# zhirui-gao/PoseProbe

Measured on AMD Instinct MI355X. Metric: rays_per_sec_train_step, higher is better.
Workload: dtype f32 (3xf16-split products); 1 GPU; DTU-scan1-like 3-view 400x400, object-branch train step (ray select, render, losses, backward, TV+Adam), 160^3 grid, 186 samples/ray, N_rand=1024/GPU; per-step ray permutation + jitter pre-generated on the host and resident in HBM (the reference draws randperm inside the step); grid=160, n_rand_per_gpu=1024, samples_in_bbox_last_step=57637, parallelism=single GPU

## Files before the change

poseprobe_amd/csrc/pp_gemm_tn_tr.h:

```cpp
#pragma once
#include "pp_gemm_split.h"

#ifndef TN_DBG
#define TN_DBG 0
#endif
__device__ __forceinline__ int tn_off(int row, int ch) { return 256 * row + 16 * (ch ^ (((row & 3) << 2) | ((row >> 2) & 3))); }

#ifdef TN_TIMERS
#define TN_TIMERS_ON 1
__device__ unsigned long long g_tn_t[8];
extern "C" int pp_debug_read_tn_timers(unsigned long long* out8, int reset) {
  if (hipMemcpyFromSymbol(out8, HIP_SYMBOL(g_tn_t), sizeof(g_tn_t)) != hipSuccess) return 1;
  if (reset) { unsigned long long z[8] = {0}; if (hipMemcpyToSymbol(HIP_SYMBOL(g_tn_t), z, sizeof(z)) != hipSuccess) return 1; }
  return 0;
}
#endif
static __global__ __launch_bounds__(256, 2) void k_gemm_tn_tr(const float* __restrict__ Y_, int ldy, const float* __restrict__ X_, int ldx,
                                                          int Kx_, float* __restrict__ Wbar_, int ldwb, float* __restrict__ bbar_,
                                                          const int32_t* __restrict__ count, int rcap,
                                                          const float* __restrict__ y_max, const float* __restrict__ x_max) {
  constexpr int CH = 64;
  __shared__ __attribute__((aligned(1024))) unsigned char img[4 * CH * 256];
  unsigned char* const Yh = img;
  unsigned char* const Yl = img + CH * 256;
  unsigned char* const Xh = img + 2 * CH * 256;
  unsigned char* const Xl = img + 3 * CH * 256;
  const int nkb = (Kx_ + 127) >> 7;
  const int nb = blockIdx.y / nkb, kb = blockIdx.y - nb * nkb;
  const float* __restrict__ Y = Y_ + nb * 128;
  const float* __restrict__ X = X_ + kb * 128;
  const int Kx = min(128, Kx_ - kb * 128);
  float* __restrict__ Wbar = Wbar_ + (size_t)nb * 128 * ldwb + kb * 128;
  float* __restrict__ bbar = (bbar_ && kb == 0) ? bbar_ + nb * 128 : nullptr;
  const int R = min(count[0], rcap);
  const int rows_per_wg = ((R + (int)gridDim.x - 1) / (int)gridDim.x + CH - 1) / CH * CH;
  const int rb = blockIdx.x * rows_per_wg;
  if (rb >= R) return;
  const int re = min(rb + rows_per_wg, R);
  const int tid = threadIdx.x, lane = tid & 63, wid = tid >> 6;
  const int wr = wid >> 1, wc = wid & 1;
  const int l31 = lane & 31, lh = lane >> 5;
  const float sY = pp_split_scale(y_max[0]), sX = pp_split_scale(x_max[0]);
  const int c4 = tid & 31, rblk = tid >> 5;
  const int kx4 = Kx >> 2;
  f32x16 acc[2][2];
#pragma unroll
  for (int t = 0; t < 2; ++t)
#pragma unroll
    for (int u = 0; u < 2; ++u)
#pragma unroll
      for (int i = 0; i < 16; ++i) acc[t][u][i] = 0.f;
  float bsum[4] = {0.f, 0.f, 0.f, 0.f};
  float4 ry[8], rx[8];
  auto load_rows = [&](int r0, int i0, int i1) {
#pragma unroll
    for (int i = 0; i < 8; ++i) {
      if (i < i0 || i >= i1) continue;
      const int gr = min(r0 + rblk * 8 + i, R - 1);
      ry[i] = *reinterpret_cast<const float4*>(Y + (size_t)gr * ldy + c4 * 4);
      if (TN_DBG & 4) rx[i] = ry[i];
      else rx[i] = *reinterpret_cast<const float4*>(X + (size_t)gr * ldx + (c4 < kx4 ? c4 : 0) * 4);
    }
  };
  typedef __fp16 tn_h4 __attribute__((vector_size(8)));
  const int fg = lane >> 4, fq = (lane & 15) >> 2, fp = lane & 3;
  auto frag = [&](const unsigned char* plane, int cb, int ks) -> pp_half8 {
    const int ch = ((cb + 16 * (fg & 1)) >> 3) + (fp >> 1);
    const int row = ks + 8 * (fg >> 1) + fq;
    const tn_h4 a = __builtin_amdgcn_ds_read_tr16_b64_v4f16((__attribute__((address_space(3))) tn_h4*)(plane + tn_off(row, ch) + 8 * (fp & 1)));
    const tn_h4 b = __builtin_amdgcn_ds_read_tr16_b64_v4f16((__attribute__((address_space(3))) tn_h4*)(plane + tn_off(row + 4, ch) + 8 * (fp & 1)));
    typedef __fp16 tn_h8 __attribute__((vector_size(16)));
    const tn_h8 v = __builtin_shufflevector(a, b, 0, 1, 2, 3, 4, 5, 6, 7);
    return __builtin_bit_cast(pp_half8, v);
  };
#ifdef TN_TIMERS_ON
  unsigned long long tsum[8] = {0}, tprev = __builtin_readcyclecounter();
#define TN_TICK(i) do { const unsigned long long t__ = __builtin_readcyclecounter(); tsum[i] += t__ - tprev; tprev = t__; } while (0)
#else
#define TN_TICK(i) do {} while (0)
#endif
  load_rows(rb, 0, 8);
  for (int r0 = rb; r0 < re; r0 += CH) {
    asm volatile("s_waitcnt vmcnt(0)" ::: "memory");
    TN_TICK(0);
#pragma unroll
    for (int i = 0; i < 8; ++i) {
      const int o = tn_off(rblk * 8 + i, c4 >> 1) + 8 * (c4 & 1);
      const float ky = (r0 + rblk * 8 + i < re) ? 1.f : 0.f, kx = (c4 < kx4) ? ky : 0.f;
      ry[i].x *= ky; ry[i].y *= ky; ry[i].z *= ky; ry[i].w *= ky;
      rx[i].x *= kx; rx[i].y *= kx; rx[i].z *= kx; rx[i].w *= kx;
      pp_half4 h, l;
      pp_split4(ry[i], sY, h, l);
      *reinterpret_cast<pp_half4*>(Yh + o) = h;
      *reinterpret_cast<pp_half4*>(Yl + o) = l;
      pp_split4(rx[i], sX, h, l);
      *reinterpret_cast<pp_half4*>(Xh + o) = h;
      *reinterpret_cast<pp_half4*>(Xl + o) = l;
    }
    if (bbar) {
#pragma unroll
      for (int i = 0; i < 8; ++i) { bsum[0] += ry[i].x; bsum[1] += ry[i].y; bsum[2] += ry[i].z; bsum[3] += ry[i].w; }
    }
    TN_TICK(1);
    __syncthreads();
    TN_TICK(2);
    if (wc * 64 < Kx) {
      pp_half8 fa[2][4], fb[2][4];
      auto fetch = [&](int par, int ks) {
#pragma unroll
        for (int t = 0; t < 2; ++t) { fa[par][2 * t] = frag(Yh, wr * 64 + t * 32, ks); fa[par][2 * t + 1] = frag(Yl, wr * 64 + t * 32, ks); }
#pragma unroll
        for (int u = 0; u < 2; ++u) { fb[par][2 * u] = frag(Xh, wc * 64 + u * 32, ks); fb[par][2 * u + 1] = frag(Xl, wc * 64 + u * 32, ks); }
      };
      fetch(0, 0);
#pragma unroll
      for (int s4 = 0; s4 < CH / 16; ++s4) {
        const int par = s4 & 1;
        if (s4 + 1 < CH / 16 && !(TN_DBG & 2)) fetch(par ^ 1, (s4 + 1) * 16);
        if (TN_DBG & 2) { for (int i = 0; i < 4; ++i) { fa[par ^ 1][i] = fa[par][i]; fb[par ^ 1][i] = fb[par][i]; } }
#pragma unroll
        for (int t = 0; t < 2; ++t) {
#pragma unroll
          for (int u = 0; u < 2; ++u) {
            acc[t][u] = __builtin_amdgcn_mfma_f32_32x32x16_f16(fa[par][2 * t + 1], fb[par][2 * u], acc[t][u], 0, 0, 0);
            acc[t][u] = __builtin_amdgcn_mfma_f32_32x32x16_f16(fa[par][2 * t], fb[par][2 * u + 1], acc[t][u], 0, 0, 0);
            acc[t][u] = __builtin_amdgcn_mfma_f32_32x32x16_f16(fa[par][2 * t], fb[par][2 * u], acc[t][u], 0, 0, 0);
          }
          if (t == 0 && !(TN_DBG & 1)) {
            __builtin_amdgcn_sched_barrier(0);
            load_rows(r0 + CH, 2 * s4, 2 * s4 + 2);
            __builtin_amdgcn_sched_barrier(0);
          }
        }
      }
    } else if (!(TN_DBG & 1)) {
      load_rows(r0 + CH, 0, 8);
    }
    TN_TICK(3);
    __syncthreads();
    TN_TICK(4);
  }
  const float inv = 1.0f / (sY * sX);
  if (wc * 64 < Kx) {
#pragma unroll
    for (int t = 0; t < 2; ++t)
#pragma unroll
      for (int u = 0; u < 2; ++u) {
        const int k = wc * 64 + u * 32 + l31;
        if (k >= Kx) continue;
#pragma unroll
        for (int reg = 0; reg < 16; ++reg) {
          const int n = wr * 64 + t * 32 + (reg & 3) + 8 * (reg >> 2) + 4 * lh;
          atomicAdd(&Wbar[(size_t)n * ldwb + k], acc[t][u][reg] * inv);
        }
      }
  }
  if (bbar) {
    float* red = reinterpret_cast<float*>(img);
#pragma unroll
    for (int j = 0; j < 4; ++j) red[rblk * 128 + c4 * 4 + j] = bsum[j];
    __syncthreads();
    if (tid < 128) {
      float sum = 0.f;
#pragma unroll
      for (int q = 0; q < 8; ++q) sum += red[q * 128 + tid];
      atomicAdd(&bbar[tid], sum);
    }
  }
#ifdef TN_TIMERS_ON
  TN_TICK(5);
  if (tid == 0)
    for (int i = 0; i < 8; ++i) atomicAdd(&g_tn_t[i], tsum[i]);
#endif
#undef TN_TICK
}
```

poseprobe_amd/csrc/pp_mlp_split.hip:

```cpp
#include "pp_common.h"
#include "pp_mlp_fused.h"
#include "pp_gemm_split.h"

typedef float f32x4 __attribute__((ext_vector_type(4)));

#define LDA 132
#define TILE_ROWS 64
#define LDH2 136
#define PLANE (TILE_ROWS * LDH2)
#ifndef MS_DBG
#define MS_DBG 0
#endif
#ifdef MS_TIMERS
__device__ unsigned long long g_ms_t[16];
extern "C" int pp_debug_read_timers(unsigned long long* out16, int reset) {
  if (hipMemcpyFromSymbol(out16, HIP_SYMBOL(g_ms_t), sizeof(g_ms_t)) != hipSuccess) return 1;
  if (reset) { unsigned long long z[16] = {0}; if (hipMemcpyToSymbol(HIP_SYMBOL(g_ms_t), z, sizeof(z)) != hipSuccess) return 1; }
  return 0;
}
#define TICK(i) do { const unsigned long long t__ = __builtin_readcyclecounter(); tsum[i] += t__ - tprev; tprev = t__; } while (0)
#else
#define TICK(i) do {} while (0)
#endif
#define PP_WAIT_VMEM() do { __builtin_amdgcn_s_waitcnt(0x0F70); asm volatile("" ::: "memory"); } while (0)

namespace {

struct SplitW { pp_half8 h[8], l[8]; };

__device__ __forceinline__ float wave_max(float v) {
#pragma unroll
  for (int o = 32; o > 0; o >>= 1) v = fmaxf(v, __shfl_xor(v, o, 64));
  return v;
}
__device__ __forceinline__ float block_max(float v, float* red, int tid, int& phase) {
  float* set = red + 16 * (phase & 1);
  ++phase;
  v = fmaxf(v, __int_as_float(__builtin_amdgcn_update_dpp(0, __float_as_int(v), 0xB1, 0xf, 0xf, true)));
  v = fmaxf(v, __int_as_float(__builtin_amdgcn_update_dpp(0, __float_as_int(v), 0x4E, 0xf, 0xf, true)));
  v = fmaxf(v, __int_as_float(__builtin_amdgcn_update_dpp(0, __float_as_int(v), 0x141, 0xf, 0xf, true)));
  v = fmaxf(v, __int_as_float(__builtin_amdgcn_update_dpp(0, __float_as_int(v), 0x140, 0xf, 0xf, true)));
  if ((tid & 15) == 0) set[tid >> 4] = v;
  __syncthreads();
  const float4 a = *reinterpret_cast<const float4*>(set), b = *reinterpret_cast<const float4*>(set + 4),
               c = *reinterpret_cast<const float4*>(set + 8), d = *reinterpret_cast<const float4*>(set + 12);
  return fmaxf(fmaxf(fmaxf(fmaxf(a.x, a.y), fmaxf(a.z, a.w)), fmaxf(fmaxf(b.x, b.y), fmaxf(b.z, b.w))),
               fmaxf(fmaxf(fmaxf(c.x, c.y), fmaxf(c.z, c.w)), fmaxf(fmaxf(d.x, d.y), fmaxf(d.z, d.w))));
}
__device__ __forceinline__ int scale_exp(float mx) {
  if (!(mx > 0.f) || !(mx < 3.0e38f)) return 0;
  int e;
  frexpf(mx, &e);
  return min(max(15 - e, -60), 60);
}
__device__ __forceinline__ float pow2(int e) { return ldexpf(1.f, e); }
__device__ __forceinline__ float tile_scale(float mx) { return pow2(scale_exp(mx)); }
__device__ __forceinline__ void split1(float x, _Float16& h, _Float16& l) {
  h = (_Float16)x;
  l = (_Float16)(x - (float)h);
}
__device__ __forceinline__ void split8(const float4& a, const float4& b, float s, pp_half8& h, pp_half8& l) {
  const float v[8] = {a.x * s, a.y * s, a.z * s, a.w * s, b.x * s, b.y * s, b.z * s, b.w * s};
#pragma unroll
  for (int i = 0; i < 8; ++i) {
    _Float16 hh, ll;
    split1(v[i], hh, ll);
    h[i] = hh; l[i] = ll;
  }
}
__device__ __forceinline__ float amax4(const float4& v) { return fmaxf(fmaxf(fabsf(v.x), fabsf(v.y)), fmaxf(fabsf(v.z), fabsf(v.w))); }
__device__ __forceinline__ float asum4(const float4& v) { return (fabsf(v.x) + fabsf(v.y)) + (fabsf(v.z) + fabsf(v.w)); }

__device__ __forceinline__ int load_w_rows_split(SplitW& w, float& l1, const float* __restrict__ W, int n, int lh, float* red,
                                                   int tid, int& phase) {
  float4 v[16];
  float mx = 0.f, sum = 0.f;
#pragma unroll
  for (int ks = 0; ks < 8; ++ks) {
    v[2 * ks] = *reinterpret_cast<const float4*>(W + (size_t)n * 128 + 16 * ks + 8 * lh);
    v[2 * ks + 1] = *reinterpret_cast<const float4*>(W + (size_t)n * 128 + 16 * ks + 8 * lh + 4);
    mx = fmaxf(mx, fmaxf(amax4(v[2 * ks]), amax4(v[2 * ks + 1])));
    sum += asum4(v[2 * ks]) + asum4(v[2 * ks + 1]);
  }
  sum += __shfl_xor(sum, 32, 64);
  const int e = scale_exp(block_max(mx, red, tid, phase));
  const float s = pow2(e);
  l1 = block_max(sum, red, tid, phase) * 1.0001f;
#pragma unroll
  for (int ks = 0; ks < 8; ++ks) split8(v[2 * ks], v[2 * ks + 1], s, w.h[ks], w.l[ks]);
  return e;
}

struct NoHook { __device__ __forceinline__ void operator()(int) const {} };
template <int KS = 8, int LD = LDH2, int PL = PLANE, class Hook = NoHook>
__device__ __forceinline__ void mma_half(const _Float16* __restrict__ rows, const SplitW& w, f32x16& acc, int l31, int lh,
                                         Hook hook = Hook()) {
  const _Float16* p = rows + l31 * LD + 8 * lh;
  pp_half8 h = *reinterpret_cast<const pp_half8*>(p), l = *reinterpret_cast<const pp_half8*>(p + PL);
#pragma unroll
  for (int ks = 0; ks < (MS_DBG == 1 ? 0 : KS); ++ks) {
    pp_half8 nh = h, nl = l;
    if (ks + 1 < KS) {
      nh = *reinterpret_cast<const pp_half8*>(p + 16 * (ks + 1));
      nl = *reinterpret_cast<const pp_half8*>(p + 16 * (ks + 1) + PL);
    }
    acc = __builtin_amdgcn_mfma_f32_32x32x16_f16(w.h[ks], l, acc, 0, 0, 0);
    acc = __builtin_amdgcn_mfma_f32_32x32x16_f16(w.l[ks], h, acc, 0, 0, 0);
    acc = __builtin_amdgcn_mfma_f32_32x32x16_f16(w.h[ks], h, acc, 0, 0, 0);
    h = nh; l = nl;
    hook(ks);
  }
}

__device__ __forceinline__ void zero16(f32x16& acc) {
#pragma unroll
  for (int i = 0; i < 16; ++i) acc[i] = 0.f;
}

typedef _Float16 half2_t __attribute__((ext_vector_type(2)));

template <int COLS, bool SPLIT>
struct HalfEpilogue {
  float4 b[4];
  float y[16];
  float p[16];
  unsigned h[8], l[8];
  float xmax;
  __device__ __forceinline__ void begin(const float* __restrict__ brow) {
    xmax = 0.f;
#pragma unroll
    for (int q = 0; q < 4; ++q) b[q] = *reinterpret_cast<const float4*>(brow + 8 * q);
  }
  __device__ __forceinline__ void step(int i, const f32x16& acc, float inv, float snext, bool ok, float* __restrict__ Crow,
                                       _Float16* __restrict__ Arow) {
    __builtin_amdgcn_sched_barrier(0);
    if (i == 0) {
#pragma unroll
      for (int q = 0; q < 4; ++q) {
        y[4 * q] = fmaf(acc[4 * q], inv, b[q].x); y[4 * q + 1] = fmaf(acc[4 * q + 1], inv, b[q].y);
        y[4 * q + 2] = fmaf(acc[4 * q + 2], inv, b[q].z); y[4 * q + 3] = fmaf(acc[4 * q + 3], inv, b[q].w);
      }
    } else if (i == 1) {
      if (COLS == 4) {
#pragma unroll
        for (int e = 0; e < 16; ++e)
          asm("v_mov_b32_dpp %0, %1 quad_perm:[0,0,0,0] row_mask:0xf bank_mask:0xf bound_ctrl:1" : "=v"(p[e]) : "v"(y[e]));
#pragma unroll
        for (int e = 0; e < 16; ++e) asm("v_ashrrev_i32 %0, 31, %1" : "=v"(p[e]) : "v"(p[e]));
      }
    } else if (i == 2) {
#pragma unroll
      for (int e = 0; e < 16; ++e) {
        if (COLS == 4) asm("v_bfi_b32 %0, %1, 0, %2" : "=v"(y[e]) : "v"(p[e]), "v"(y[e]));
        else y[e] = fmaxf(y[e], 0.f);
      }
// ... 896 lines not shown
    const int r0 = t * TILE_ROWS;
    float gl = 0.f;
    if (tid < 192) {
      const int m = tid / 3, o = tid - 3 * m;
      const float r = RG[b][0][tid];
      gl = (r0 + m < R) ? RG[b][1][tid] * r * (1.f - r) : 0.f;
      GL[m * 4 + o] = gl;
      if (logit_grad && r0 + m < R) logit_grad[(size_t)(r0 + m) * lg_ld + o] = gl;
    } else {
      GL[(tid - 192) * 4 + 3] = 0.f;
    }
    slot_max(&Mx[b][4], fabsf(gl), lane);
  };
  auto w3_accumulate = [&]() {
    const float* __restrict__ xs = &XS[(h0 * 32) * 128 + j0];
#pragma unroll 8
    for (int r = 0; r < 32; ++r) {
      const float4 g = *reinterpret_cast<const float4*>(&GL[(h0 * 32 + r) * 4]);
      const float x = xs[r * 128];
      wacc3[0] = fmaf(g.x, x, wacc3[0]); wacc3[1] = fmaf(g.y, x, wacc3[1]); wacc3[2] = fmaf(g.z, x, wacc3[2]);
      if (j0 < 3) bacc3 += GL[(h0 * 32 + r) * 4 + j0];
    }
  };
  int e2n = 0;
  auto out_layer_bwd = [&](int t, int b, _Float16* dst) {
    const float gmx = slot_get(&Mx[b][4]);
    const int eg = scale_exp(gmx);
    const int e2 = scale_exp(gmx * w3l1);
    const float sg = pow2(eg), s2 = pow2(e2), inv = pow2(-(eg + ew3)), n2 = pow2(-e2);
    const int r0 = t * TILE_ROWS;
    float* crow = ybar + (size_t)(r0 + l31) * 128 + fb;
    HalfEpilogueB<true> eb;
#pragma unroll
    for (int hh = 0; hh < 2; ++hh) {
      float4 x = *reinterpret_cast<const float4*>(&GL[(hh * 32 + l31) * 4]);
      if (lh != 0) x = make_float4(0.f, 0.f, 0.f, 0.f);
      pp_half8 xh, xl;
      split8(x, make_float4(0.f, 0.f, 0.f, 0.f), sg, xh, xl);
      f32x16 a;
      zero16(a);
      a = __builtin_amdgcn_mfma_f32_32x32x16_f16(a3h, xl, a, 0, 0, 0);
      a = __builtin_amdgcn_mfma_f32_32x32x16_f16(a3l, xh, a, 0, 0, 0);
      a = __builtin_amdgcn_mfma_f32_32x32x16_f16(a3h, xh, a, 0, 0, 0);
      eb.begin(&XS[(hh * 32 + l31) * 128 + fb]);
      eb.all(a, inv, s2, r0 + hh * 32 + l31 < R, crow + hh * 32 * 128, dst + (hh * 32 + l31) * LDH2 + fb);
      slot_max(&Mx[b][hh], eb.vmax(n2), lane);
    }
    e2n = e2;
  };

  if (tid < 16) Mx[tid >> 3][tid & 7] = 0u;
  stage(blockIdx.x, 0);
  __builtin_amdgcn_s_waitcnt(0);
  __syncthreads();
  logit_grads(blockIdx.x, 0);
  __syncthreads();
  w3_accumulate();
  out_layer_bwd(blockIdx.x, 0, At[0]);
  __syncthreads();

  int par = 0;
  for (int tile = blockIdx.x; tile < ntiles; tile += gridDim.x, par ^= 1) {
    const int r0 = tile * TILE_ROWS;
    const int tnext = tile + gridDim.x;
    const bool more = tnext < ntiles;
    const bool ok0 = r0 + l31 < R, ok1 = r0 + 32 + l31 < R;
    _Float16* const Aa = At[par];
    _Float16* const Ab = At[par ^ 1];
    const int e2 = e2n;
    float* const crow = ybar + (size_t)(r0 + l31) * 128 + fb;
    f32x16 acc0, acc1;
    HalfEpilogueB<true> eb;
    if (tid < 5) Mx[par ^ 1][tid] = 0u;
    if (more) stage(tnext, par ^ 1);
    stage_tile(H1, r0, GT);
    zero16(acc0);
    mma_half(Aa, w2, acc0, l31, lh);
    PP_WAIT_VMEM();
    __syncthreads();
    const int e10 = scale_exp(slot_get(&Mx[par][0]) * l1_2), e11 = scale_exp(slot_get(&Mx[par][1]) * l1_2);
    zero16(acc1);
    eb.begin(&GT[l31 * 128 + fb]);
    mma_half(Aa + 32 * LDH2, w2, acc1, l31, lh, [&](int ks) {
      eb.step(ks, acc0, pow2(-(e2 + ew2)), pow2(e10), ok0, crow + LS, Ab + l31 * LDH2 + fb);
    });
    slot_max(&Mx[par][2], eb.vmax(pow2(-e10)), lane);
    __syncthreads();
    zero16(acc0);
    eb.begin(&GT[(32 + l31) * 128 + fb]);
    mma_half(Ab, w1, acc0, l31, lh, [&](int ks) {
      eb.step(ks, acc1, pow2(-(e2 + ew2)), pow2(e11), ok1, crow + LS + 32 * 128, Ab + (32 + l31) * LDH2 + fb);
    });
    slot_max(&Mx[par][3], eb.vmax(pow2(-e11)), lane);
    __syncthreads();
    stage_tile(H0, r0, GT);
    zero16(acc1);
    mma_half(Ab + 32 * LDH2, w1, acc1, l31, lh);
    PP_WAIT_VMEM();
    __syncthreads();
    const int e00 = scale_exp(slot_get(&Mx[par][2]) * l1_1), e01 = scale_exp(slot_get(&Mx[par][3]) * l1_1);
    eb.begin(&GT[l31 * 128 + fb]);
    eb.all(acc0, pow2(-(e10 + ew1)), pow2(e00), ok0, crow + 2 * LS, Aa + l31 * LDH2 + fb);
    eb.begin(&GT[(32 + l31) * 128 + fb]);
    eb.all(acc1, pow2(-(e11 + ew1)), pow2(e01), ok1, crow + 2 * LS + 32 * 128, Aa + (32 + l31) * LDH2 + fb);
    if (more) logit_grads(tnext, par ^ 1);
    __syncthreads();
    {
      f32x16 fa;
      zero16(fa);
      mma_half(Aa + rb * 32 * LDH2, w0, fa, l31, lh);
      const float inv = pow2(-((rb ? e01 : e00) + ew0));
      const int row = r0 + rb * 32 + l31;
      if (row < R) {
        float* __restrict__ ft = feat_grad + (size_t)row * 64 + (wid & 1) * 32 + 4 * lh;
#pragma unroll
        for (int q = 0; q < 4; ++q)
          *reinterpret_cast<float4*>(ft + 8 * q) = make_float4(fa[4 * q] * inv, fa[4 * q + 1] * inv, fa[4 * q + 2] * inv, fa[4 * q + 3] * inv);
      }
    }
    if (more) {
      w3_accumulate();
      out_layer_bwd(tnext, par ^ 1, Ab);
    }
    __syncthreads();
  }

  float* red = reinterpret_cast<float*>(At[0]);
  __syncthreads();
  if (h0 == 1) {
#pragma unroll
    for (int o = 0; o < 3; ++o) red[o * 128 + j0] = wacc3[o];
    if (j0 < 3) red[4 * 128 + j0] = bacc3;
  }
  __syncthreads();
  if (h0 == 0) {
#pragma unroll
    for (int o = 0; o < 3; ++o) atomicAdd(&params_grad[RGF_W3 + o * 128 + j0], wacc3[o] + red[o * 128 + j0]);
    if (j0 < 3) atomicAdd(&params_grad[RGF_B3 + j0], bacc3 + red[4 * 128 + j0]);
  }
}

int pp_launch_rgb_fused_bwd_s(const float* params, const float* acts, const float* rgb, const float* rgb_grad,
                              const int32_t* count, int capacity, float* ybar, float* params_grad, float* feat_grad,
                              float* logit_grad, int lg_ld, hipStream_t st) {
  const int ntiles = pp_div_up(capacity, TILE_ROWS);
  const int grid = ntiles < PP_FUSED_WGS ? ntiles : PP_FUSED_WGS;
  hipLaunchKernelGGL(k_rgb_fused_bwd_s, dim3(grid), dim3(256), 0, st, params, acts, rgb, rgb_grad, count, capacity, ybar,
                     params_grad, feat_grad, logit_grad, lg_ld);
  return 0;
}

namespace {

template <int KX>
__device__ __forceinline__ void wgs_issue_piece(const WgradOperands& L, int r0, int R, float* Ybuf, float* Xbuf, int wid, int lane, int i) {
  const int l31 = lane & 31, lh = lane >> 5;
  {
    const int rl = 16 * wid + 2 * i;
    const int row = min(r0 + rl + lh, R - 1);
    __builtin_amdgcn_global_load_lds(PP_GLOBAL_PTR(L.Y + (size_t)row * 128 + l31 * 4), PP_LDS_PTR(Ybuf + rl * 128), 16, 0, 0);
  }
  if (KX == 128) {
    const int rl = 16 * wid + 2 * i;
    const int row = min(r0 + rl + lh, R - 1);
    __builtin_amdgcn_global_load_lds(PP_GLOBAL_PTR(L.X + (size_t)row * 128 + l31 * 4), PP_LDS_PTR(Xbuf + rl * 128), 16, 0, 0);
  } else if (i < 4) {
    const int l15 = lane & 15, lq = lane >> 4;
    const int rl = 16 * wid + 4 * i;
    const int row = min(r0 + rl + lq, R - 1);
    __builtin_amdgcn_global_load_lds(PP_GLOBAL_PTR(L.X + (size_t)row * 64 + l15 * 4), PP_LDS_PTR(Xbuf + rl * 64), 16, 0, 0);
  }
}
template <int KX>
__device__ __forceinline__ void wgs_issue(const WgradOperands& L, int r0, int R, float* Ybuf, float* Xbuf, int wid, int lane) {
#pragma unroll
  for (int i = 0; i < 8; ++i) wgs_issue_piece<KX>(L, r0, R, Ybuf, Xbuf, wid, lane, i);
}

__device__ __forceinline__ void frag_split(const float (&v)[8], float s, pp_half8& h, pp_half8& l) {
  unsigned hh[4], ll[4];
#pragma unroll
  for (int k = 0; k < 4; ++k) {
    const float x0 = v[2 * k] * s, x1 = v[2 * k + 1] * s;
    asm("v_cvt_pk_f16_f32 %0, %1, %2" : "=v"(hh[k]) : "v"(x0), "v"(x1));
    asm("v_fma_mixlo_f16 %0, %1, -1.0, %2 op_sel_hi:[1,0,0]" : "=v"(ll[k]) : "v"(hh[k]), "v"(x0));
    asm("v_fma_mixhi_f16 %0, %1, -1.0, %2 op_sel:[1,0,0] op_sel_hi:[1,0,0]" : "+v"(ll[k]) : "v"(hh[k]), "v"(x1));
  }
  typedef unsigned u4 __attribute__((ext_vector_type(4)));
  const u4 hv = {hh[0], hh[1], hh[2], hh[3]}, lv = {ll[0], ll[1], ll[2], ll[3]};
  h = __builtin_bit_cast(pp_half8, hv);
  l = __builtin_bit_cast(pp_half8, lv);
}

struct WgsLayer {
  int eY, eX;
  float bsum[2];
};

template <int NF>
__device__ __forceinline__ bool frag_exceeds(const float (&v)[NF][8], float lim, float& m) {
  m = 0.f;
#pragma unroll
  for (int f = 0; f < NF; ++f)
#pragma unroll
    for (int k = 0; k < 4; ++k) asm("v_max3_f32 %0, |%1|, |%2|, %0" : "+v"(m) : "v"(v[f][2 * k]), "v"(v[f][2 * k + 1]));
  return __builtin_amdgcn_ballot_w64(m > lim) != 0ull;
}

template <int KX, int CSTEP, class Issue>
__device__ __forceinline__ void wgs_compute(const float* __restrict__ Ybuf, const float* __restrict__ Xbuf, f32x16 (&acc)[2][KX / 64],
                                            WgsLayer& st, bool bias, int wr, int wc, int l31, int lh, Issue issue) {
  constexpr int NB = KX / 64;
  float sY = pow2(st.eY), sX = pow2(st.eX), limY = pow2(15 - st.eY), limX = pow2(15 - st.eX);
  const float* yp = Ybuf + (8 * lh) * 128 + 64 * wr + l31;
  const float* xp = Xbuf + (8 * lh) * KX + 32 * NB * wc + l31;
  float ry[2][8], rx[NB][8];
  pp_half8 ah[2] = {}, al[2] = {}, bh[NB] = {}, bl[NB] = {};
  auto rescale = [&](int d) {
    const float f = pow2(d);
#pragma unroll
    for (int t = 0; t < 2; ++t)
#pragma unroll
      for (int u = 0; u < NB; ++u)
#pragma unroll
        for (int i = 0; i < 16; ++i) acc[t][u][i] *= f;
  };
#pragma unroll
  for (int ks = -1; ks < 4; ++ks) {
    pp_half8 ch[2] = {ah[0], ah[1]}, cl[2] = {al[0], al[1]}, dh[NB], dl[NB];
#pragma unroll
    for (int u = 0; u < NB; ++u) { dh[u] = bh[u]; dl[u] = bl[u]; }
    __builtin_amdgcn_sched_barrier(0);
    if (ks < 3) {
#pragma unroll
      for (int t = 0; t < 2; ++t)
#pragma unroll
        for (int j = 0; j < 8; ++j) ry[t][j] = yp[(16 * (ks + 1) + j) * 128 + 32 * t];
#pragma unroll
      for (int u = 0; u < NB; ++u)
#pragma unroll
        for (int j = 0; j < 8; ++j) rx[u][j] = xp[(16 * (ks + 1) + j) * KX + 32 * u];
    }
    __builtin_amdgcn_sched_barrier(0);
    if (ks >= 0) {
#pragma unroll
      for (int u = 0; u < NB; ++u) {
        acc[0][u] = __builtin_amdgcn_mfma_f32_32x32x16_f16(cl[0], dh[u], acc[0][u], 0, 0, 0);
        acc[0][u] = __builtin_amdgcn_mfma_f32_32x32x16_f16(ch[0], dl[u], acc[0][u], 0, 0, 0);
        acc[0][u] = __builtin_amdgcn_mfma_f32_32x32x16_f16(ch[0], dh[u], acc[0][u], 0, 0, 0);
      }
    }
    __builtin_amdgcn_sched_barrier(0);
    if (ks >= 0 && ks < 2) { issue(4 * ks); issue(4 * ks + 1); issue(4 * ks + 2); issue(4 * ks + 3); }
    __builtin_amdgcn_sched_barrier(0);
    if (ks >= 0) {
#pragma unroll
      for (int u = 0; u < NB; ++u) {
        acc[1][u] = __builtin_amdgcn_mfma_f32_32x32x16_f16(cl[1], dh[u], acc[1][u], 0, 0, 0);
        acc[1][u] = __builtin_amdgcn_mfma_f32_32x32x16_f16(ch[1], dl[u], acc[1][u], 0, 0, 0);
        acc[1][u] = __builtin_amdgcn_mfma_f32_32x32x16_f16(ch[1], dh[u], acc[1][u], 0, 0, 0);
      }
    }
    __builtin_amdgcn_sched_barrier(0);
    if (ks < 3) {
      float m;
      if (frag_exceeds<2>(ry, limY, m)) {
        const int e = scale_exp(wave_max(m)) - 2;
        rescale(e - st.eY);
        st.eY = e; sY = pow2(e); limY = pow2(15 - e);
      }
      if (frag_exceeds<NB>(rx, limX, m)) {
        const int e = scale_exp(wave_max(m)) - 2;
        rescale(e - st.eX);
        st.eX = e; sX = pow2(e); limX = pow2(15 - e);
      }
#pragma unroll
      for (int t = 0; t < 2; ++t) {
        if (bias) {
#pragma unroll
          for (int j = 0; j < 8; j += CSTEP) st.bsum[t] += ry[t][j];
        }
        frag_split(ry[t], sY, ah[t], al[t]);
      }
#pragma unroll
      for (int u = 0; u < NB; ++u) frag_split(rx[u], sX, bh[u], bl[u]);
    }
    __builtin_amdgcn_sched_barrier(0);
  }
}

}

template <int KX, int CSTEP>
__device__ __forceinline__ void wgs_layer(const WgradOperands& L, int R, int ntiles, int wg, int nwg, float* __restrict__ Yb0,
                                          float* __restrict__ Xb0, float* __restrict__ Yb1, float* __restrict__ Xb1) {
  constexpr int NB = KX / 64;
  const int tid = threadIdx.x, lane = tid & 63, wid = tid >> 6;
  const int wr = wid >> 1, wc = wid & 1, l31 = lane & 31, lh = lane >> 5;
  f32x16 acc[2][NB];
#pragma unroll
  for (int t = 0; t < 2; ++t)
#pragma unroll
    for (int u = 0; u < NB; ++u) zero16(acc[t][u]);
  WgsLayer st = {60, 60, {0.f, 0.f}};
  const bool bias = L.bbar != nullptr && wc == 0;
  auto prepare = [&](int r0, float* Ybuf) {
    if (r0 + TILE_ROWS > R) {
      for (int i = tid; i < TILE_ROWS * 128; i += 256)
        if (r0 + (i >> 7) >= R) Ybuf[i] = 0.f;
      __syncthreads();
    }
  };
  const int first = ntiles - 1 - wg;
  wgs_issue<KX>(L, first * TILE_ROWS, R, Yb0, Xb0, wid, lane);
#ifdef MS_TIMERS
  unsigned long long tsum[16] = {0}, tprev = __builtin_readcyclecounter();
#endif
  for (int t0 = first; t0 >= 0; t0 -= 2 * nwg) {
    const int t1 = t0 - nwg, t2 = t1 - nwg;
    TICK(4);
    PP_WAIT_VMEM(); __syncthreads();
    TICK(0);
    prepare(t0 * TILE_ROWS, Yb0);
    TICK(1);
    TICK(2);
    wgs_compute<KX, CSTEP>(Yb0, Xb0, acc, st, bias, wr, wc, l31, lh, [&](int i) {
      if (t1 >= 0) wgs_issue_piece<KX>(L, t1 * TILE_ROWS, R, Yb1, Xb1, wid, lane, i);
    });
    TICK(3);
    if (t1 < 0) break;
    PP_WAIT_VMEM(); __syncthreads();
    TICK(0);
    prepare(t1 * TILE_ROWS, Yb1);
    TICK(1);
    TICK(2);
    wgs_compute<KX, CSTEP>(Yb1, Xb1, acc, st, bias, wr, wc, l31, lh, [&](int i) {
      if (t2 >= 0) wgs_issue_piece<KX>(L, t2 * TILE_ROWS, R, Yb0, Xb0, wid, lane, i);
    });
    TICK(3);
  }
#ifdef MS_TIMERS
  if (tid == 0)
    for (int i = 0; i < 16; ++i) atomicAdd(&g_ms_t[i], tsum[i]);
#endif
  const float f = pow2(-(st.eY + st.eX));
#pragma unroll
  for (int t = 0; t < 2; ++t)
#pragma unroll
    for (int u = 0; u < NB; ++u) {
      const int k = 32 * NB * wc + u * 32 + l31;
#pragma unroll
      for (int reg = 0; reg < 16; ++reg) {
        const int n = wr * 64 + t * 32 + (reg & 3) + 8 * (reg >> 2) + 4 * lh;
        atomicAdd(&L.Wbar[(size_t)n * KX + k], acc[t][u][reg] * f);
      }
    }
  if (bias) {
#pragma unroll
    for (int t = 0; t < 2; ++t) {
      const float v = st.bsum[t] + __shfl_xor(st.bsum[t], 32, 64);
      if (lh == 0) atomicAdd(&L.bbar[64 * wr + 32 * t + l31], v);
    }
  }
}

template <int KXC, int CSTEP>
__global__ __launch_bounds__(256) void k_wgrad_chain_s(WgradOperands LA, WgradOperands LB, WgradOperands LC,
                                                       const int32_t* __restrict__ count, int rmul, int rcap, int nwg_ab, int nwg_c) {
  __shared__ __attribute__((aligned(16))) float Yb0[TILE_ROWS * 128];
  __shared__ __attribute__((aligned(16))) float Xb0[TILE_ROWS * 128];
  __shared__ __attribute__((aligned(16))) float Yb1[TILE_ROWS * 128];
  __shared__ __attribute__((aligned(16))) float Xb1[TILE_ROWS * 128];
  const int R = min(count[0] * rmul, rcap);
  const int ntiles = (R + TILE_ROWS - 1) / TILE_ROWS;
  const int bx = blockIdx.x;
  const int layer = bx < nwg_ab ? 0 : (bx < 2 * nwg_ab ? 1 : 2);
  const int wg = bx - layer * nwg_ab, nwg = layer < 2 ? nwg_ab : nwg_c;
  if (wg >= ntiles) return;
  const WgradOperands L = layer == 0 ? LA : (layer == 1 ? LB : LC);
  if (KXC == 128 || layer < 2) wgs_layer<128, CSTEP>(L, R, ntiles, wg, nwg, Yb0, Xb0, Yb1, Xb1);
  else wgs_layer<KXC, CSTEP>(L, R, ntiles, wg, nwg, Yb0, Xb0, Yb1, Xb1);
}

int pp_launch_wgrad_chain_s(const float* YA, const float* XA, float* WA, const float* YB, const float* XB, float* WB,
                            const float* YC, const float* XC, float* WC, int kxc, const int32_t* count, int rmul, int rcap,
                            hipStream_t st, float* bA, float* bB, float* bC, int wgs_) {
  WgradOperands LA{YA, XA, WA, bA}, LB{YB, XB, WB, bB}, LC{YC, XC, WC, bC};
  const int ntiles = pp_div_up(rcap, TILE_ROWS);
  const int wgs = wgs_ > 0 ? (wgs_ < 16 ? 16 : wgs_) : PP_FUSED_WGS;
  int nab = kxc == 128 ? wgs / 3 : (wgs * 4) / 11, nc = kxc == 128 ? wgs / 3 : wgs - 2 * ((wgs * 4) / 11);
  if (nab > ntiles) nab = ntiles;
  if (nc > ntiles) nc = ntiles;
  if (kxc == 128)
    hipLaunchKernelGGL((k_wgrad_chain_s<128, 4>), dim3(2 * nab + nc), dim3(256), 0, st, LA, LB, LC, count, rmul, rcap, nab, nc);
  else
    hipLaunchKernelGGL((k_wgrad_chain_s<64, 1>), dim3(2 * nab + nc), dim3(256), 0, st, LA, LB, LC, count, rmul, rcap, nab, nc);
  return 0;
}
```

Before: 973,500 rays/s.

## Rework fused wgrad chain to split-once LDS image with transposed reads

The chained weight-gradient kernel used to stage raw fp32 tiles in LDS through global_load_lds and split every fragment into hi/lo halves per wave. It now loads rows into registers, splits each element into fp16 hi/lo once, and stores them into a swizzled LDS image. Waves then read fragments with ds_read_tr16, sharing code with the TN GEMM through a new header. Dynamic rescaling moves to a workgroup-wide check with LDS flags, and tail rows are spread evenly across workgroups. The kernel also targets two blocks per CU and launches twice as many workgroups, halving them at runtime when there are few tiles. This cuts redundant conversion work and improves load balance, but adds extra barriers and atomics and possible re-conversion when the scale changes.

```diff
diff --git a/poseprobe_amd/csrc/pp_gemm_tn_tr.h b/poseprobe_amd/csrc/pp_gemm_tn_tr.h
--- a/poseprobe_amd/csrc/pp_gemm_tn_tr.h
+++ b/poseprobe_amd/csrc/pp_gemm_tn_tr.h
@@ -1,10 +1,9 @@
 #pragma once
-#include "pp_gemm_split.h"
+#include "pp_split_image.h"
 
 #ifndef TN_DBG
 #define TN_DBG 0
 #endif
-__device__ __forceinline__ int tn_off(int row, int ch) { return 256 * row + 16 * (ch ^ (((row & 3) << 2) | ((row >> 2) & 3))); }
 
 #ifdef TN_TIMERS
 #define TN_TIMERS_ON 1
@@ -62,17 +61,7 @@
       else rx[i] = *reinterpret_cast<const float4*>(X + (size_t)gr * ldx + (c4 < kx4 ? c4 : 0) * 4);
     }
   };
-  typedef __fp16 tn_h4 __attribute__((vector_size(8)));
-  const int fg = lane >> 4, fq = (lane & 15) >> 2, fp = lane & 3;
-  auto frag = [&](const unsigned char* plane, int cb, int ks) -> pp_half8 {
-    const int ch = ((cb + 16 * (fg & 1)) >> 3) + (fp >> 1);
-    const int row = ks + 8 * (fg >> 1) + fq;
-    const tn_h4 a = __builtin_amdgcn_ds_read_tr16_b64_v4f16((__attribute__((address_space(3))) tn_h4*)(plane + tn_off(row, ch) + 8 * (fp & 1)));
-    const tn_h4 b = __builtin_amdgcn_ds_read_tr16_b64_v4f16((__attribute__((address_space(3))) tn_h4*)(plane + tn_off(row + 4, ch) + 8 * (fp & 1)));
-    typedef __fp16 tn_h8 __attribute__((vector_size(16)));
-    const tn_h8 v = __builtin_shufflevector(a, b, 0, 1, 2, 3, 4, 5, 6, 7);
-    return __builtin_bit_cast(pp_half8, v);
-  };
+  auto frag = [&](const unsigned char* plane, int cb, int ks) { return tn_frag(plane, cb, ks, lane); };
 #ifdef TN_TIMERS_ON
   unsigned long long tsum[8] = {0}, tprev = __builtin_readcyclecounter();
 #define TN_TICK(i) do { const unsigned long long t__ = __builtin_readcyclecounter(); tsum[i] += t__ - tprev; tprev = t__; } while (0)
@@ -85,17 +74,11 @@
     TN_TICK(0);
 #pragma unroll
     for (int i = 0; i < 8; ++i) {
-      const int o = tn_off(rblk * 8 + i, c4 >> 1) + 8 * (c4 & 1);
       const float ky = (r0 + rblk * 8 + i < re) ? 1.f : 0.f, kx = (c4 < kx4) ? ky : 0.f;
       ry[i].x *= ky; ry[i].y *= ky; ry[i].z *= ky; ry[i].w *= ky;
       rx[i].x *= kx; rx[i].y *= kx; rx[i].z *= kx; rx[i].w *= kx;
-      pp_half4 h, l;
-      pp_split4(ry[i], sY, h, l);
-      *reinterpret_cast<pp_half4*>(Yh + o) = h;
-      *reinterpret_cast<pp_half4*>(Yl + o) = l;
-      pp_split4(rx[i], sX, h, l);
-      *reinterpret_cast<pp_half4*>(Xh + o) = h;
-      *reinterpret_cast<pp_half4*>(Xl + o) = l;
+      tn_store4(Yh, Yl, rblk * 8 + i, c4, ry[i], sY);
+      tn_store4(Xh, Xl, rblk * 8 + i, c4, rx[i], sX);
     }
     if (bbar) {
 #pragma unroll
diff --git a/poseprobe_amd/csrc/pp_mlp_split.hip b/poseprobe_amd/csrc/pp_mlp_split.hip
--- a/poseprobe_amd/csrc/pp_mlp_split.hip
+++ b/poseprobe_amd/csrc/pp_mlp_split.hip
@@ -1,6 +1,7 @@
 #include "pp_common.h"
 #include "pp_mlp_fused.h"
 #include "pp_gemm_split.h"
+#include "pp_split_image.h"
 
 typedef float f32x4 __attribute__((ext_vector_type(4)));
 
@@ -1203,198 +1204,166 @@
 
 namespace {
 
-template <int KX>
-__device__ __forceinline__ void wgs_issue_piece(const WgradOperands& L, int r0, int R, float* Ybuf, float* Xbuf, int wid, int lane, int i) {
-  const int l31 = lane & 31, lh = lane >> 5;
-  {
-    const int rl = 16 * wid + 2 * i;
-    const int row = min(r0 + rl + lh, R - 1);
-    __builtin_amdgcn_global_load_lds(PP_GLOBAL_PTR(L.Y + (size_t)row * 128 + l31 * 4), PP_LDS_PTR(Ybuf + rl * 128), 16, 0, 0);
-  }
-  if (KX == 128) {
-    const int rl = 16 * wid + 2 * i;
-    const int row = min(r0 + rl + lh, R - 1);
-    __builtin_amdgcn_global_load_lds(PP_GLOBAL_PTR(L.X + (size_t)row * 128 + l31 * 4), PP_LDS_PTR(Xbuf + rl * 128), 16, 0, 0);
-  } else if (i < 4) {
-    const int l15 = lane & 15, lq = lane >> 4;
-    const int rl = 16 * wid + 4 * i;
-    const int row = min(r0 + rl + lq, R - 1);
-    __builtin_amdgcn_global_load_lds(PP_GLOBAL_PTR(L.X + (size_t)row * 64 + l15 * 4), PP_LDS_PTR(Xbuf + rl * 64), 16, 0, 0);
-  }
-}
-template <int KX>
-__device__ __forceinline__ void wgs_issue(const WgradOperands& L, int r0, int R, float* Ybuf, float* Xbuf, int wid, int lane) {
-#pragma unroll
-  for (int i = 0; i < 8; ++i) wgs_issue_piece<KX>(L, r0, R, Ybuf, Xbuf, wid, lane, i);
-}
-
-__device__ __forceinline__ void frag_split(const float (&v)[8], float s, pp_half8& h, pp_half8& l) {
-  unsigned hh[4], ll[4];
-#pragma unroll
-  for (int k = 0; k < 4; ++k) {
-    const float x0 = v[2 * k] * s, x1 = v[2 * k + 1] * s;
-    asm("v_cvt_pk_f16_f32 %0, %1, %2" : "=v"(hh[k]) : "v"(x0), "v"(x1));
-    asm("v_fma_mixlo_f16 %0, %1, -1.0, %2 op_sel_hi:[1,0,0]" : "=v"(ll[k]) : "v"(hh[k]), "v"(x0));
-    asm("v_fma_mixhi_f16 %0, %1, -1.0, %2 op_sel:[1,0,0] op_sel_hi:[1,0,0]" : "+v"(ll[k]) : "v"(hh[k]), "v"(x1));
-  }
-  typedef unsigned u4 __attribute__((ext_vector_type(4)));
-  const u4 hv = {hh[0], hh[1], hh[2], hh[3]}, lv = {ll[0], ll[1], ll[2], ll[3]};
-  h = __builtin_bit_cast(pp_half8, hv);
-  l = __builtin_bit_cast(pp_half8, lv);
-}
-
-struct WgsLayer {
-  int eY, eX;
-  float bsum[2];
-};
-
-template <int NF>
-__device__ __forceinline__ bool frag_exceeds(const float (&v)[NF][8], float lim, float& m) {
-  m = 0.f;
-#pragma unroll
-  for (int f = 0; f < NF; ++f)
-#pragma unroll
-    for (int k = 0; k < 4; ++k) asm("v_max3_f32 %0, |%1|, |%2|, %0" : "+v"(m) : "v"(v[f][2 * k]), "v"(v[f][2 * k + 1]));
-  return __builtin_amdgcn_ballot_w64(m > lim) != 0ull;
-}
-
-template <int KX, int CSTEP, class Issue>
-__device__ __forceinline__ void wgs_compute(const float* __restrict__ Ybuf, const float* __restrict__ Xbuf, f32x16 (&acc)[2][KX / 64],
-                                            WgsLayer& st, bool bias, int wr, int wc, int l31, int lh, Issue issue) {
+struct WgsUnit { int r0, rend; };
+
+__device__ __forceinline__ WgsUnit wgs_unit(int k, int full, int wg, int nwg, int ntiles, int R, int rem_rows, int q) {
+  if (k < full) {
+    const int t = ntiles - 1 - wg - k * nwg;
+    return {t * TILE_ROWS, R};
+  }
+  const int hi = rem_rows - wg * q;
+  return {max(hi - q, 0), hi};
+}
+
+template <int KX, int CSTEP>
+__device__ __forceinline__ void wgs_layer(const WgradOperands& L, int R, int ntiles, int wg, int nwg, unsigned char* __restrict__ img,
+                                          float2* __restrict__ flags) {
   constexpr int NB = KX / 64;
-  float sY = pow2(st.eY), sX = pow2(st.eX), limY = pow2(15 - st.eY), limX = pow2(15 - st.eX);
-  const float* yp = Ybuf + (8 * lh) * 128 + 64 * wr + l31;
-  const float* xp = Xbuf + (8 * lh) * KX + 32 * NB * wc + l31;
-  float ry[2][8], rx[NB][8];
-  pp_half8 ah[2] = {}, al[2] = {}, bh[NB] = {}, bl[NB] = {};
-  auto rescale = [&](int d) {
-    const float f = pow2(d);
-#pragma unroll
-    for (int t = 0; t < 2; ++t)
-#pragma unroll
-      for (int u = 0; u < NB; ++u)
-#pragma unroll
-        for (int i = 0; i < 16; ++i) acc[t][u][i] *= f;
-  };
-#pragma unroll
-  for (int ks = -1; ks < 4; ++ks) {
-    pp_half8 ch[2] = {ah[0], ah[1]}, cl[2] = {al[0], al[1]}, dh[NB], dl[NB];
-#pragma unroll
-    for (int u = 0; u < NB; ++u) { dh[u] = bh[u]; dl[u] = bl[u]; }
-    __builtin_amdgcn_sched_barrier(0);
-    if (ks < 3) {
-#pragma unroll
-      for (int t = 0; t < 2; ++t)
-#pragma unroll
-        for (int j = 0; j < 8; ++j) ry[t][j] = yp[(16 * (ks + 1) + j) * 128 + 32 * t];
-#pragma unroll
-      for (int u = 0; u < NB; ++u)
-#pragma unroll
-        for (int j = 0; j < 8; ++j) rx[u][j] = xp[(16 * (ks + 1) + j) * KX + 32 * u];
-    }
-    __builtin_amdgcn_sched_barrier(0);
-    if (ks >= 0) {
-#pragma unroll
-      for (int u = 0; u < NB; ++u) {
-        acc[0][u] = __builtin_amdgcn_mfma_f32_32x32x16_f16(cl[0], dh[u], acc[0][u], 0, 0, 0);
-        acc[0][u] = __builtin_amdgcn_mfma_f32_32x32x16_f16(ch[0], dl[u], acc[0][u], 0, 0, 0);
-        acc[0][u] = __builtin_amdgcn_mfma_f32_32x32x16_f16(ch[0], dh[u], acc[0][u], 0, 0, 0);
-      }
-    }
-    __builtin_amdgcn_sched_barrier(0);
-    if (ks >= 0 && ks < 2) { issue(4 * ks); issue(4 * ks + 1); issue(4 * ks + 2); issue(4 * ks + 3); }
-    __builtin_amdgcn_sched_barrier(0);
-    if (ks >= 0) {
-#pragma unroll
-      for (int u = 0; u < NB; ++u) {
-        acc[1][u] = __builtin_amdgcn_mfma_f32_32x32x16_f16(cl[1], dh[u], acc[1][u], 0, 0, 0);
-        acc[1][u] = __builtin_amdgcn_mfma_f32_32x32x16_f16(ch[1], dl[u], acc[1][u], 0, 0, 0);
-        acc[1][u] = __builtin_amdgcn_mfma_f32_32x32x16_f16(ch[1], dh[u], acc[1][u], 0, 0, 0);
-      }
-    }
-    __builtin_amdgcn_sched_barrier(0);
-    if (ks < 3) {
-      float m;
-      if (frag_exceeds<2>(ry, limY, m)) {
-        const int e = scale_exp(wave_max(m)) - 2;
-        rescale(e - st.eY);
-        st.eY = e; sY = pow2(e); limY = pow2(15 - e);
-      }
-      if (frag_exceeds<NB>(rx, limX, m)) {
-        const int e = scale_exp(wave_max(m)) - 2;
-        rescale(e - st.eX);
-        st.eX = e; sX = pow2(e); limX = pow2(15 - e);
-      }
-#pragma unroll
-      for (int t = 0; t < 2; ++t) {
-        if (bias) {
-#pragma unroll
-          for (int j = 0; j < 8; j += CSTEP) st.bsum[t] += ry[t][j];
-        }
-        frag_split(ry[t], sY, ah[t], al[t]);
-      }
-#pragma unroll
-      for (int u = 0; u < NB; ++u) frag_split(rx[u], sX, bh[u], bl[u]);
-    }
-    __builtin_amdgcn_sched_barrier(0);
-  }
-}
-
-}
-
-template <int KX, int CSTEP>
-__device__ __forceinline__ void wgs_layer(const WgradOperands& L, int R, int ntiles, int wg, int nwg, float* __restrict__ Yb0,
-                                          float* __restrict__ Xb0, float* __restrict__ Yb1, float* __restrict__ Xb1) {
-  constexpr int NB = KX / 64;
+  constexpr int XR = KX / 16;
+  constexpr int XC = KX / 4;
+  const int full = ntiles / nwg;
+  const int rem_rows = min((ntiles - full * nwg) * TILE_ROWS, R);
+  const int q = ((rem_rows + nwg - 1) / nwg + 15) & ~15;
+  const int nunits = full + (rem_rows - wg * q > 0 ? 1 : 0);
+  if (nunits == 0) return;
+  unsigned char* const Yh = img;
+  unsigned char* const Yl = img + TILE_ROWS * 256;
+  unsigned char* const Xh = img + 2 * TILE_ROWS * 256;
+  unsigned char* const Xl = img + 3 * TILE_ROWS * 256;
   const int tid = threadIdx.x, lane = tid & 63, wid = tid >> 6;
   const int wr = wid >> 1, wc = wid & 1, l31 = lane & 31, lh = lane >> 5;
+  const int c4 = tid & 31, rblk = tid >> 5;
+  const int xc4 = c4 % XC, xrow = 8 * rblk + (c4 / XC) * XR;
+  const bool bias = L.bbar != nullptr;
   f32x16 acc[2][NB];
 #pragma unroll
   for (int t = 0; t < 2; ++t)
 #pragma unroll
     for (int u = 0; u < NB; ++u) zero16(acc[t][u]);
-  WgsLayer st = {60, 60, {0.f, 0.f}};
-  const bool bias = L.bbar != nullptr && wc == 0;
-  auto prepare = [&](int r0, float* Ybuf) {
-    if (r0 + TILE_ROWS > R) {
-      for (int i = tid; i < TILE_ROWS * 128; i += 256)
-        if (r0 + (i >> 7) >= R) Ybuf[i] = 0.f;
-      __syncthreads();
-    }
-  };
-  const int first = ntiles - 1 - wg;
-  wgs_issue<KX>(L, first * TILE_ROWS, R, Yb0, Xb0, wid, lane);
-#ifdef MS_TIMERS
-  unsigned long long tsum[16] = {0}, tprev = __builtin_readcyclecounter();
-#endif
-  for (int t0 = first; t0 >= 0; t0 -= 2 * nwg) {
-    const int t1 = t0 - nwg, t2 = t1 - nwg;
-    TICK(4);
-    PP_WAIT_VMEM(); __syncthreads();
-    TICK(0);
-    prepare(t0 * TILE_ROWS, Yb0);
-    TICK(1);
-    TICK(2);
-    wgs_compute<KX, CSTEP>(Yb0, Xb0, acc, st, bias, wr, wc, l31, lh, [&](int i) {
-      if (t1 >= 0) wgs_issue_piece<KX>(L, t1 * TILE_ROWS, R, Yb1, Xb1, wid, lane, i);
-    });
-    TICK(3);
-    if (t1 < 0) break;
-    PP_WAIT_VMEM(); __syncthreads();
-    TICK(0);
-    prepare(t1 * TILE_ROWS, Yb1);
-    TICK(1);
-    TICK(2);
-    wgs_compute<KX, CSTEP>(Yb1, Xb1, acc, st, bias, wr, wc, l31, lh, [&](int i) {
-      if (t2 >= 0) wgs_issue_piece<KX>(L, t2 * TILE_ROWS, R, Yb0, Xb0, wid, lane, i);
-    });
-    TICK(3);
-  }
-#ifdef MS_TIMERS
-  if (tid == 0)
-    for (int i = 0; i < 16; ++i) atomicAdd(&g_ms_t[i], tsum[i]);
-#endif
-  const float f = pow2(-(st.eY + st.eX));
+  float bsum[4] = {0.f, 0.f, 0.f, 0.f};
+  int eY = 60, eX = 60;
+  float sY = pow2(eY), sX = pow2(eX), limY = pow2(15 - eY), limX = pow2(15 - eX);
+
+  float4 ry[8], rx[XR];
+  auto load_rows = [&](int r0, int i0, int i1) {
+#pragma unroll
+    for (int i = 0; i < 8; ++i) {
+      if (i < i0 || i >= i1) continue;
+      ry[i] = *reinterpret_cast<const float4*>(L.Y + (size_t)min(r0 + 8 * rblk + i, R - 1) * 128 + c4 * 4);
+      if (i < XR) rx[i] = *reinterpret_cast<const float4*>(L.X + (size_t)min(r0 + xrow + i, R - 1) * KX + xc4 * 4);
+    }
+  };
+  auto mask = [&](const WgsUnit& u) {
+    if (u.r0 + TILE_ROWS > u.rend) {
+      const float4 z = make_float4(0.f, 0.f, 0.f, 0.f);
+#pragma unroll
+      for (int i = 0; i < 8; ++i) if (u.r0 + 8 * rblk + i >= u.rend) ry[i] = z;
+#pragma unroll
+      for (int i = 0; i < XR; ++i) if (u.r0 + xrow + i >= u.rend) rx[i] = z;
+    }
+  };
+  auto check = [&](float2* set) {
+    float my = 0.f, mx = 0.f;
+#pragma unroll
+    for (int i = 0; i < 8; ++i) my = fmaxf(my, amax4(ry[i]));
+#pragma unroll
+    for (int i = 0; i < XR; ++i) mx = fmaxf(mx, amax4(rx[i]));
+    float py = 0.f, px = 0.f;
+    if (__builtin_amdgcn_ballot_w64(my > limY) != 0ull) py = wave_max(my);
+    if (__builtin_amdgcn_ballot_w64(mx > limX) != 0ull) px = wave_max(mx);
+    if (lane == 0) set[wid] = make_float2(py, px);
+  };
+  auto adopt = [&](const float2* set) -> int {
+    const float4 a = *reinterpret_cast<const float4*>(set), b = *reinterpret_cast<const float4*>(set + 2);
+    const float my = fmaxf(fmaxf(a.x, a.z), fmaxf(b.x, b.z)), mx = fmaxf(fmaxf(a.y, a.w), fmaxf(b.y, b.w));
+    if (!(my > 0.f) && !(mx > 0.f)) return 0;
+    int d = 0, changed = 0;
+    if (my > 0.f) { const int e = scale_exp(my) - 2; d += e - eY; eY = e; changed |= 1; }
+    if (mx > 0.f) { const int e = scale_exp(mx) - 2; d += e - eX; eX = e; changed |= 2; }
+    sY = pow2(eY); sX = pow2(eX); limY = pow2(15 - eY); limX = pow2(15 - eX);
+    const float f = pow2(d);
+#pragma unroll
+    for (int t = 0; t < 2; ++t)
+#pragma unroll
+      for (int u = 0; u < NB; ++u)
+#pragma unroll
+        for (int i = 0; i < 16; ++i) acc[t][u][i] *= f;
+    return changed;
+  };
+  auto convert = [&](bool y, bool x) {
+    if (y) {
+#pragma unroll
+      for (int i = 0; i < 8; ++i) tn_store4(Yh, Yl, 8 * rblk + i, c4, ry[i], sY);
+    }
+    if (x) {
+#pragma unroll
+      for (int i = 0; i < XR; ++i) tn_store4(Xh, Xl, xrow + i, xc4, rx[i], sX);
+    }
+  };
+  auto frag = [&](const unsigned char* plane, int cb, int ks) { return tn_frag(plane, cb, ks, lane); };
+
+  WgsUnit cur = wgs_unit(0, full, wg, nwg, ntiles, R, rem_rows, q);
+  load_rows(cur.r0, 0, 8);
+  PP_WAIT_VMEM();
+  mask(cur);
+  check(flags + 4);
+  __syncthreads();
+  adopt(flags + 4);
+  for (int k = 0; k < nunits; ++k) {
+    const bool has_next = k + 1 < nunits;
+    const WgsUnit nxt = has_next ? wgs_unit(k + 1, full, wg, nwg, ntiles, R, rem_rows, q) : cur;
+    if (k > 0) {
+      PP_WAIT_VMEM();
+      mask(cur);
+    }
+    check(flags);
+    convert(true, true);
+    if (bias) {
+#pragma unroll
+      for (int i = 0; i < 8; i += CSTEP) { bsum[0] += ry[i].x; bsum[1] += ry[i].y; bsum[2] += ry[i].z; bsum[3] += ry[i].w; }
+    }
+    __syncthreads();
+    {
+      const int changed = adopt(flags);
+      if (changed) {
+        convert(changed & 1, changed & 2);
+        __syncthreads();
+      }
+    }
+    const int ng = (min(cur.rend - cur.r0, TILE_ROWS) + 15) >> 4;
+    pp_half8 fa[2][4], fb[2][2 * NB];
+    auto fetch = [&](int par, int ks) {
+#pragma unroll
+      for (int t = 0; t < 2; ++t) { fa[par][2 * t] = frag(Yh, wr * 64 + t * 32, ks); fa[par][2 * t + 1] = frag(Yl, wr * 64 + t * 32, ks); }
+#pragma unroll
+      for (int u = 0; u < NB; ++u) { fb[par][2 * u] = frag(Xh, 32 * NB * wc + u * 32, ks); fb[par][2 * u + 1] = frag(Xl, 32 * NB * wc + u * 32, ks); }
+    };
+    fetch(0, 0);
+#pragma unroll
+    for (int s4 = 0; s4 < TILE_ROWS / 16; ++s4) {
+      const int par = s4 & 1;
+      if (s4 + 1 < ng) fetch(par ^ 1, (s4 + 1) * 16);
+#pragma unroll
+      for (int t = 0; t < 2; ++t) {
+        if (s4 < ng) {
+#pragma unroll
+          for (int u = 0; u < NB; ++u) {
+            acc[t][u] = __builtin_amdgcn_mfma_f32_32x32x16_f16(fa[par][2 * t + 1], fb[par][2 * u], acc[t][u], 0, 0, 0);
+            acc[t][u] = __builtin_amdgcn_mfma_f32_32x32x16_f16(fa[par][2 * t], fb[par][2 * u + 1], acc[t][u], 0, 0, 0);
+            acc[t][u] = __builtin_amdgcn_mfma_f32_32x32x16_f16(fa[par][2 * t], fb[par][2 * u], acc[t][u], 0, 0, 0);
+          }
+        }
+        if (t == 0 && has_next) {
+          __builtin_amdgcn_sched_barrier(0);
+          load_rows(nxt.r0, 2 * s4, 2 * s4 + 2);
+          __builtin_amdgcn_sched_barrier(0);
+        }
+      }
+    }
+    __syncthreads();
+    cur = nxt;
+  }
+  const float f = pow2(-(eY + eX));
 #pragma unroll
   for (int t = 0; t < 2; ++t)
 #pragma unroll
@@ -1407,30 +1376,39 @@
       }
     }
   if (bias) {
-#pragma unroll
-    for (int t = 0; t < 2; ++t) {
-      const float v = st.bsum[t] + __shfl_xor(st.bsum[t], 32, 64);
-      if (lh == 0) atomicAdd(&L.bbar[64 * wr + 32 * t + l31], v);
-    }
-  }
+    float* red = reinterpret_cast<float*>(img);
+#pragma unroll
+    for (int j = 0; j < 4; ++j) red[rblk * 128 + c4 * 4 + j] = bsum[j];
+    __syncthreads();
+    if (tid < 128) {
+      float sum = 0.f;
+#pragma unroll
+      for (int i = 0; i < 8; ++i) sum += red[i * 128 + tid];
+      atomicAdd(&L.bbar[tid], sum);
+    }
+  }
+}
+
 }
 
 template <int KXC, int CSTEP>
-__global__ __launch_bounds__(256) void k_wgrad_chain_s(WgradOperands LA, WgradOperands LB, WgradOperands LC,
-                                                       const int32_t* __restrict__ count, int rmul, int rcap, int nwg_ab, int nwg_c) {
-  __shared__ __attribute__((aligned(16))) float Yb0[TILE_ROWS * 128];
-  __shared__ __attribute__((aligned(16))) float Xb0[TILE_ROWS * 128];
-  __shared__ __attribute__((aligned(16))) float Yb1[TILE_ROWS * 128];
-  __shared__ __attribute__((aligned(16))) float Xb1[TILE_ROWS * 128];
+__global__ __launch_bounds__(256, 2) void k_wgrad_chain_s(WgradOperands LA, WgradOperands LB, WgradOperands LC,
+                                                          const int32_t* __restrict__ count, int rmul, int rcap, int nwg_ab, int nwg_c) {
+  __shared__ __attribute__((aligned(1024))) unsigned char img[4 * TILE_ROWS * 256];
+  __shared__ __attribute__((aligned(16))) float2 flags[8];
   const int R = min(count[0] * rmul, rcap);
   const int ntiles = (R + TILE_ROWS - 1) / TILE_ROWS;
+  if (ntiles < 8 * nwg_ab) {
+    nwg_ab = max(nwg_ab / 2, 1);
+    nwg_c = max(nwg_c / 2, 1);
+  }
   const int bx = blockIdx.x;
+  if (bx >= 2 * nwg_ab + nwg_c) return;
   const int layer = bx < nwg_ab ? 0 : (bx < 2 * nwg_ab ? 1 : 2);
   const int wg = bx - layer * nwg_ab, nwg = layer < 2 ? nwg_ab : nwg_c;
-  if (wg >= ntiles) return;
   const WgradOperands L = layer == 0 ? LA : (layer == 1 ? LB : LC);
-  if (KXC == 128 || layer < 2) wgs_layer<128, CSTEP>(L, R, ntiles, wg, nwg, Yb0, Xb0, Yb1, Xb1);
-  else wgs_layer<KXC, CSTEP>(L, R, ntiles, wg, nwg, Yb0, Xb0, Yb1, Xb1);
+  if (KXC == 128 || layer < 2) wgs_layer<128, CSTEP>(L, R, ntiles, wg, nwg, img, flags);
+  else wgs_layer<KXC, CSTEP>(L, R, ntiles, wg, nwg, img, flags);
 }
 
 int pp_launch_wgrad_chain_s(const float* YA, const float* XA, float* WA, const float* YB, const float* XB, float* WB,
@@ -1438,7 +1416,7 @@
                             hipStream_t st, float* bA, float* bB, float* bC, int wgs_) {
   WgradOperands LA{YA, XA, WA, bA}, LB{YB, XB, WB, bB}, LC{YC, XC, WC, bC};
   const int ntiles = pp_div_up(rcap, TILE_ROWS);
-  const int wgs = wgs_ > 0 ? (wgs_ < 16 ? 16 : wgs_) : PP_FUSED_WGS;
+  const int wgs = 2 * (wgs_ > 0 ? (wgs_ < 16 ? 16 : wgs_) : PP_FUSED_WGS);
   int nab = kxc == 128 ? wgs / 3 : (wgs * 4) / 11, nc = kxc == 128 ? wgs / 3 : wgs - 2 * ((wgs * 4) / 11);
   if (nab > ntiles) nab = ntiles;
   if (nc > ntiles) nc = ntiles;
diff --git a/poseprobe_amd/csrc/pp_split_image.h b/poseprobe_amd/csrc/pp_split_image.h
--- /dev/null
+++ b/poseprobe_amd/csrc/pp_split_image.h
@@ -0,0 +1,24 @@
+#pragma once
+#include "pp_gemm_split.h"
+
+__device__ __forceinline__ int tn_off(int row, int ch) { return 256 * row + 16 * (ch ^ (((row & 3) << 2) | ((row >> 2) & 3))); }
+
+__device__ __forceinline__ void tn_store4(unsigned char* hi, unsigned char* lo, int row, int c4, float4 x, float s) {
+  const int o = tn_off(row, c4 >> 1) + 8 * (c4 & 1);
+  pp_half4 h, l;
+  pp_split4(x, s, h, l);
+  *reinterpret_cast<pp_half4*>(hi + o) = h;
+  *reinterpret_cast<pp_half4*>(lo + o) = l;
+}
+
+__device__ __forceinline__ pp_half8 tn_frag(const unsigned char* plane, int cb, int ks, int lane) {
+  typedef __fp16 tn_h4 __attribute__((vector_size(8)));
+  typedef __fp16 tn_h8 __attribute__((vector_size(16)));
+  const int fg = lane >> 4, fq = (lane & 15) >> 2, fp = lane & 3;
+  const int ch = ((cb + 16 * (fg & 1)) >> 3) + (fp >> 1);
+  const int row = ks + 8 * (fg >> 1) + fq;
+  const tn_h4 a = __builtin_amdgcn_ds_read_tr16_b64_v4f16((__attribute__((address_space(3))) tn_h4*)(plane + tn_off(row, ch) + 8 * (fp & 1)));
+  const tn_h4 b = __builtin_amdgcn_ds_read_tr16_b64_v4f16((__attribute__((address_space(3))) tn_h4*)(plane + tn_off(row + 4, ch) + 8 * (fp & 1)));
+  const tn_h8 v = __builtin_shufflevector(a, b, 0, 1, 2, 3, 4, 5, 6, 7);
+  return __builtin_bit_cast(pp_half8, v);
+}
```

Result: faster. 991,000 rays/s (median of 6 runs) (+1.8%).
